# aligokalppeker/hypelcnn

Hardware: AMD Instinct MI355X
Metric: HSI+LiDAR patches/sec fwd+bwd (GRSS2013 7×7×145) at 1/2/4/8 GPU (higher is better)
Workload: dtype f32 (3 x bf16 split operands, 6 partial products, fp32 accumulate); 1 GPU; BASELINE.json configs[1]: GRSS2013 HYPELCNNModel, batch 1024 per GPU, fp32 HIP kernels; train step (fwd+bwd+TF1-Adam), 7x7 patch, 144 HSI + 1 LiDAR bands, 15 classes, alg_param_hypelcnn.json, random-init weights; batch_per_gpu=1024, global_batch=1024, parallelism=single, hip_graph=True

## Files before the change

### hypelcnn_amd/csrc/elementwise.hip

```cpp
#include <stdlib.h>

#include "common.h"


namespace {

constexpr int STAT_TX = 64;

struct EwShape {
    int tx_log2;
    int grid;
};
static inline EwShape ew_shape(int64_t rows, int cvec) {
    int l = 0;
    while ((1 << l) < cvec && l < 8) ++l;
    const int ty = 256 >> l;
    int64_t g = (rows + ty - 1) / ty;
    if (g < 1) g = 1;
    constexpr int cap = 8192;
    if (g > cap) g = cap;
    return EwShape{l, (int)g};
}
static inline bool aligned16(const void* p) { return p == nullptr || (((uintptr_t)p) & 15) == 0; }
static inline bool rows_v4(const void* p, int64_t ld) { return p == nullptr || (aligned16(p) && ld % 4 == 0); }
// ... 351 lines not shown
        const double unbiased = n_total > 1.0 ? m2 / (n_total - 1.0) : var;
        moving_mean[col] = (float)((double)moving_mean[col] * decay + mean_a * (1.0 - (double)decay));
        moving_var[col] = (float)((double)moving_var[col] * decay + unbiased * (1.0 - (double)decay));
    }
}

template <int VEC>
__global__ __launch_bounds__(256) void col_stats_partial_kernel(const float* __restrict__ x, int64_t ld, int64_t rows,
                                                                 int c, int chunk_rows, float* __restrict__ partial) {
    constexpr int TX = STAT_TX / VEC, TY = 256 / TX;
    __shared__ float sh[2][TY][STAT_TX];
    const int tx = threadIdx.x & (TX - 1), ty = threadIdx.x / TX;
    const int col = blockIdx.y * STAT_TX + tx * VEC;
    const int64_t r0 = (int64_t)blockIdx.x * chunk_rows;
    const int64_t r1 = min(rows, r0 + (int64_t)chunk_rows);
    Vec<VEC> s = {}, ss = {}, shift = {};
    if (col < c) {
        shift.load(x + r0 * ld + col);
#pragma unroll 4
        for (int64_t r = r0 + ty; r < r1; r += TY) {
            Vec<VEC> v;
            v.load(x + r * ld + col);
            vec_each<VEC>([&](int k) {
                const float d = v.v[k] - shift.v[k];
                s.v[k] += d;
                ss.v[k] += d * d;
            });
        }
    }
    s.store(&sh[0][ty][tx * VEC]);
    ss.store(&sh[1][ty][tx * VEC]);
    __syncthreads();
    const int cc = blockIdx.y * STAT_TX + threadIdx.x;
    if (threadIdx.x < STAT_TX && cc < c) {
        float ts = 0.0f, tss = 0.0f;
#pragma unroll
        for (int k = 0; k < TY; ++k) {
            ts += sh[0][k][threadIdx.x];
            tss += sh[1][k][threadIdx.x];
        }
        const float cnt = (float)(r1 - r0);
        const float mean_d = ts / cnt;
        float m2 = tss - ts * mean_d;
        if (m2 < 0.0f) m2 = 0.0f;
        float shift_cc;
        if constexpr (VEC == 1) shift_cc = shift.v[0];
        else shift_cc = x[r0 * ld + cc];
        float* po = partial + (int64_t)blockIdx.x * 2 * c;
        po[cc] = shift_cc + mean_d;
        po[c + cc] = m2;
    }
}

__global__ void rstd_from_var_kernel(const float* __restrict__ var, int c, float eps, float* __restrict__ rstd) {
    const int i = blockIdx.x * blockDim.x + threadIdx.x;
    if (i < c) rstd[i] = (float)(1.0 / sqrt((double)var[i] + (double)eps));
}

template <int VEC>
__global__ __launch_bounds__(256) void bn_act_fwd_kernel(
    const float* __restrict__ y, int64_t ldy, int64_t rows, int c, const float* __restrict__ mean,
    const float* __restrict__ rstd, const float* __restrict__ beta, int act, float alpha,
    const float* __restrict__ mask, int64_t ldm, const float* __restrict__ res1, int64_t ld1,
    const int32_t* __restrict__ idx1, const float* __restrict__ res2, int64_t ld2, const int32_t* __restrict__ idx2,
    float* __restrict__ z, int64_t ldz, int tx_log2) {
    ew_loop<VEC>(rows, c, tx_log2, [&](int64_t row, int col) {
        Vec<VEC> v;
        v.load(y + row * ldy + col);
        if (mean) {
            Vec<VEC> m, r, b;
            m.load_param(mean + col); r.load_param(rstd + col); b.load_param(beta + col);
#pragma unroll
            for (int k = 0; k < VEC; ++k) v.v[k] = hypel_bn_pre(hypel_bn_xhat(v.v[k], m.v[k], r.v[k]), b.v[k]);
        }
#pragma unroll
        for (int k = 0; k < VEC; ++k) v.v[k] = hypel_act(v.v[k], act, alpha);
        if (mask) {
            Vec<VEC> mk;
            mk.load(mask + row * ldm + col);
#pragma unroll
            for (int k = 0; k < VEC; ++k) v.v[k] *= mk.v[k];
        }
        if (res1) {
            if (idx1) {
#pragma unroll
                for (int k = 0; k < VEC; ++k) v.v[k] += res1[row * ld1 + idx1[col + k]];
            } else {
                Vec<VEC> t;
                t.load(res1 + row * ld1 + col);
#pragma unroll
                for (int k = 0; k < VEC; ++k) v.v[k] += t.v[k];
            }
        }
        if (res2) {
            if (idx2) {
#pragma unroll
                for (int k = 0; k < VEC; ++k) v.v[k] += res2[row * ld2 + idx2[col + k]];
            } else {
                Vec<VEC> t;
                t.load(res2 + row * ld2 + col);
#pragma unroll
                for (int k = 0; k < VEC; ++k) v.v[k] += t.v[k];
            }
        }
        v.store(z + row * ldz + col);
    });
// ... 727 lines not shown
                                            int32_t n_splits, int32_t accumulate, hypel_stream_t stream) {
    HYPEL_REQUIRE(partial0 && out0 && partial1 && out1 && n_splits >= 1 && count0 > 0 && count1 > 0,
                  "hypel_reduce_splits_pair_f32");
    if (n_splits >= 32 && count0 <= 65536 && count1 <= 65536) {
        hipLaunchKernelGGL(reduce_splits_wave_pair_kernel, dim3(hypel_grid_1d((count0 + count1) * 64, 256)), dim3(256), 0, ST,
                           partial0, stride0, count0, out0, partial1, stride1, count1, out1, n_splits, accumulate);
        HYPEL_CHECK_LAUNCH("hypel_reduce_splits_pair_f32");
        return 0;
    }
    int rc = hypel_reduce_splits_f32(partial0, stride0, n_splits, out0, count0, accumulate, nullptr, 0, 0, stream);
    if (rc == 0) rc = hypel_reduce_splits_f32(partial1, stride1, n_splits, out1, count1, accumulate, nullptr, 0, 0, stream);
    return rc;
}

extern "C" int hypel_reduce_splits_multi_f32(const float* base, const hypel_reduce_entry_t* entries, int32_t n_entries,
                                             hypel_stream_t stream) {
    HYPEL_REQUIRE(base && entries && n_entries >= 0, "hypel_reduce_splits_multi_f32");
    if (n_entries == 0) return 0;
    constexpr int gx = 768;
    hipLaunchKernelGGL(reduce_splits_multi_kernel, dim3(gx, n_entries), dim3(256), 0, ST, base, entries);
    HYPEL_CHECK_LAUNCH("hypel_reduce_splits_multi_f32");
    return 0;
}

extern "C" int hypel_reduce_splits_multi_sized_f32(const float* base, const hypel_reduce_entry_t* entries, int32_t n_entries,
                                                   int64_t max_count, hypel_stream_t stream) {
    HYPEL_REQUIRE(base && entries && n_entries >= 0 && max_count >= 0, "hypel_reduce_splits_multi_sized_f32");
    if (n_entries == 0 || max_count == 0) return 0;
    const int64_t want = (max_count + 4 * 256 - 1) / (4 * 256);
    const int gx = (int)(want < 1 ? 1 : (want > 768 ? 768 : want));
    hipLaunchKernelGGL(reduce_splits_multi_kernel, dim3(gx, n_entries), dim3(256), 0, ST, base, entries);
    HYPEL_CHECK_LAUNCH("hypel_reduce_splits_multi_sized_f32");
    return 0;
}

static int launch_col_stats(const float* x, int64_t ld, int64_t rows, int32_t c, int32_t chunk_rows, float* partial,
                            hypel_stream_t stream) {
    const int n_chunks = (int)((rows + chunk_rows - 1) / chunk_rows);
    const bool v4 = c % 4 == 0 && rows_v4(x, ld);
    hipLaunchKernelGGL(HYPEL_VEC_KERNEL(v4, col_stats_partial_kernel), dim3(n_chunks, (c + STAT_TX - 1) / STAT_TX), dim3(256),
                       0, ST, x, ld, rows, c, chunk_rows, partial);
    return 0;
}

extern "C" int hypel_col_stats_partial(const float* x, int64_t ld, int64_t rows, int32_t c, int32_t chunk_rows,
                                       float* partial, hypel_stream_t stream) {
    HYPEL_REQUIRE(x && partial && rows > 0 && c > 0 && chunk_rows > 0, "hypel_col_stats_partial");
    launch_col_stats(x, ld, rows, c, chunk_rows, partial,
                     stream);
    HYPEL_CHECK_LAUNCH("hypel_col_stats_partial");
    return 0;
}

extern "C" int hypel_bn_finalize(const float* partial, int32_t n_chunks, int32_t chunk_rows, int64_t rows, int32_t c,
                                 float eps, float* mean, float* rstd, float* moving_mean, float* moving_var,
                                 float decay, hypel_stream_t stream) {
    HYPEL_REQUIRE(partial && mean && rstd && n_chunks > 0 && c > 0, "hypel_bn_finalize");
    HYPEL_REQUIRE((moving_mean == nullptr) == (moving_var == nullptr), "hypel_bn_finalize");
    hipLaunchKernelGGL(bn_finalize_kernel, dim3((c + 15) / 16), dim3(256), 0, ST, partial, n_chunks, chunk_rows, rows,
                       c, eps, mean, rstd, moving_mean, moving_var, decay);
    HYPEL_CHECK_LAUNCH("hypel_bn_finalize");
    return 0;
}

extern "C" int hypel_bn_merge_partials(const float* partial, int32_t n_chunks, int32_t chunk_rows, int64_t rows,
                                       int32_t c, float* out, hypel_stream_t stream) {
    HYPEL_REQUIRE(partial && out && n_chunks > 0 && c > 0 && rows > 0, "hypel_bn_merge_partials");
    hipLaunchKernelGGL(bn_merge_partials_kernel, dim3((c + 15) / 16), dim3(256), 0, ST, partial, n_chunks, chunk_rows,
                       rows, c, out);
    HYPEL_CHECK_LAUNCH("hypel_bn_merge_partials");
    return 0;
}

extern "C" int hypel_bn_finalize_ranks(const float* gathered, int32_t world, int32_t c, float eps, float* mean,
                                       float* rstd, float* moving_mean, float* moving_var, float decay,
                                       hypel_stream_t stream) {
    HYPEL_REQUIRE(gathered && mean && rstd && world > 0 && c > 0, "hypel_bn_finalize_ranks");
    HYPEL_REQUIRE((moving_mean == nullptr) == (moving_var == nullptr), "hypel_bn_finalize_ranks");
    hipLaunchKernelGGL(bn_finalize_ranks_kernel, dim3((c + 63) / 64), dim3(64), 0, ST, gathered, world, c, eps, mean,
                       rstd, moving_mean, moving_var, decay);
    HYPEL_CHECK_LAUNCH("hypel_bn_finalize_ranks");
    return 0;
}

extern "C" int hypel_rstd_from_var(const float* var, int32_t c, float eps, float* rstd, hypel_stream_t stream) {
    HYPEL_REQUIRE(var && rstd && c > 0, "hypel_rstd_from_var");
    hipLaunchKernelGGL(rstd_from_var_kernel, dim3((c + 63) / 64), dim3(64), 0, ST, var, c, eps, rstd);
    HYPEL_CHECK_LAUNCH("hypel_rstd_from_var");
    return 0;
}

extern "C" int hypel_bn_act_fwd(const float* y, int64_t ldy, int64_t rows, int32_t c, const float* mean,
                                const float* rstd, const float* beta, int32_t act, float alpha, const float* mask,
                                int64_t ldm, const float* res1, int64_t ld1, const int32_t* idx1, const float* res2,
                                int64_t ld2, const int32_t* idx2, float* z, int64_t ldz, hypel_stream_t stream) {
    HYPEL_REQUIRE(y && z && rows > 0 && c > 0, "hypel_bn_act_fwd");
    HYPEL_REQUIRE((mean == nullptr) == (rstd == nullptr) && (mean == nullptr) == (beta == nullptr), "hypel_bn_act_fwd");
    const bool v4 = c % 4 == 0 && rows_v4(y, ldy) && rows_v4(z, ldz) && rows_v4(mask, ldm) &&
                    (idx1 || rows_v4(res1, ld1)) && (idx2 || rows_v4(res2, ld2));
    const EwShape sh = ew_shape(rows, v4 ? c / 4 : c);
    hipLaunchKernelGGL(HYPEL_VEC_KERNEL(v4, bn_act_fwd_kernel), dim3(sh.grid), dim3(256), 0, ST, y, ldy, rows, c, mean,
                       rstd, beta, act, alpha, mask, ldm, res1, ld1, idx1, res2, ld2, idx2, z, ldz, sh.tx_log2);
    HYPEL_CHECK_LAUNCH("hypel_bn_act_fwd");
    return 0;
}

// ... 273 lines not shown
```

### hypelcnn_amd/plan.py

```python
import os

import numpy as np

from . import abi, graph as G
from .backend import COPY_BLOCK_DTYPE, GEMM_BM, MTILE_DTYPE, REDUCE_ENTRY_DTYPE, SEG_DTYPE, Ref
from .gemm_tables import SEG_PAIR_FLAG, GemmTables, Launch

STAT_CHUNK_ROWS = 256
STAT_BLOCKS = 256


def stat_chunk_rows(rows):
    c = (rows + STAT_BLOCKS - 1) // STAT_BLOCKS
    c = max(16, min(STAT_CHUNK_ROWS, c))
    return (c + 3) // 4 * 4
WGRAD_ROW_CHUNK = 512
TARGET_BLOCKS = 1536
WGRAD_MAX_SPLITS = 64
WGRAD_MIN_SPLITS = 0
DGRAD_MAX_SEGS = 18
MAX_TAPS_PER_TILE = 9
L2_CHUNK_BYTES = int(3.5 * (1 << 20))
SPLITK_BELOW = 400
SPLITK_TARGET = 768
TAP_SPLIT_MIN_BATCH = 64


ACT_IN_GEMM = True
SMALL_BN_ROWS = 1024
MERGE_WGRAD = True


class Storage:

    def __init__(self, buf, nb, ld, pixmap, ch_off, c, npix):
        self.buf = buf
        self.nb = nb
        self.ld = ld
        self.pixmap = pixmap
        self.ch_off = ch_off
        self.c = c
        self.npix = npix

    def pix_off(self, p):
        q = p if self.pixmap is None else self.pixmap[p]
        return q * self.nb * self.ld + self.ch_off

    @property
    def contiguous(self):
        return self.pixmap is None

    @property
    def rows(self):
        return self.npix * self.nb


MSE_PARTIALS = abi.const("HYPEL_MSE_PARTIALS")
DP_SYNC_WORK = 0.5
DP_TWO_BUCKET_BYTES = int(float(os.environ.get("HYPEL_DP_TWO_BUCKET_MB", "1048576")) * (1 << 20))
DP_BUCKET_BYTES = int(float(os.environ.get("HYPEL_DP_BUCKET_MB", "256")) * (1 << 20))
DP_MAX_BUCKETS = 8
HINT_OVERRIDE = {k: int(v) for k, v in (kv.split("=") for kv in os.environ.get("HYPEL_HINT_OVERRIDE", "").split(",") if kv)}
RESIDENT_BLOCKS_64 = 6 * 256
GEMM_SINGLE_SEG = abi.const("HYPEL_GEMM_SINGLE_SEG")
GEMM_PAIRED_SEGS = abi.const("HYPEL_GEMM_PAIRED_SEGS")
GEMM_BK = 32
GEMM_SPLIT6 = abi.const("HYPEL_GEMM_SPLIT6")
GEMM_MULTI_SPLIT6 = abi.const("HYPEL_GEMM_MULTI_SPLIT6")
_gs = os.environ.get("HYPEL_GEMM_SPLIT", "6").split(":")
GEMM_SPLIT = int(_gs[0] or 0)
GEMM_SPLIT_WIDTH = int(_gs[1]) if len(_gs) > 1 else 0
GEMM_SPLIT_MIN_FLOPS = float(os.environ.get("HYPEL_GEMM_SPLIT_MIN_GFLOP", "2")) * 1e9
SPLIT_NOMINAL_BATCH = 1024
SPLIT_NOMINAL_BATCH_GAN = 4096
GEMM_SPLIT_MIN_N = 32
SPLIT_OVERRIDE = {k: int(v) for k, v in (kv.split("=") for kv in os.environ.get("HYPEL_SPLIT_OVERRIDE", "").split(",") if kv)}
KSLICE_MIN_GAIN = 0.10
KSLICE_OVERHEAD_K = 24
KSLICE_MIN_K = 48
KSLICE_MAX_SLICES = 16
KSLICE_FRAC_MIN = 0.7
KSLICE_REDUCE_COST_K = 55
KSLICE_SLOTS = {1: 768, 2: 512, 3: 512}
SPLIT6_BN = {1: 32, 2: 64, 3: 128}
GEMM_MFMA16X4 = abi.const("HYPEL_GEMM_MFMA16X4")
GEMM_VAR_N = abi.const("HYPEL_GEMM_VAR_N")
MERGE_LEVELS = set(x for x in os.environ.get("HYPEL_MERGE_LEVELS", "fwd,dgrad,wgrad").split(",") if x and x != "0")
MERGE_LEVELS_MAX_COUT = 64
MERGE_PASS_MAX_COUT = {"fwd": 16, "dgrad": 1 << 20, "wgrad": 1 << 20}
MERGE_WGRAD_MIN_COUT = 1
MERGE_WGRAD_MAX_COUT = 64
MERGE_FWD_MAX_COUT_SPLIT = 32
MERGE_MAX_TAPS = 0
MERGE_SPLIT_MAX_TAPS = 16
MERGE_SPLIT_KPARTS = False
MERGE_FWD_HINT = 2


for _kv in filter(None, os.environ.get("HYPEL_PLAN_SET", "").split(",")):
    _k, _, _v = _kv.partition("=")
    if not isinstance(globals().get(_k), (bool, int, float)) or _k.startswith("_"):
        raise ValueError(f"HYPEL_PLAN_SET: {_k!r} is not a numeric constant of hypelcnn_amd.plan")
    globals()[_k] = type(globals()[_k])(float(_v)) if not isinstance(globals()[_k], bool) else bool(int(_v))


class TowerPlan:

    _defer_bias_sums = False

    def __init__(self, tower, nb, session, loss=None, labels_c=None, external_masks=False, seed=1234, global_nb=None,
                 sync_bn=False):
        self.tower = tower
        self.nb = int(nb)
        self.global_nb = global_nb
        dist_ = getattr(session, "dist", None)
        self.sync_bn = bool(sync_bn) and dist_ is not None and tower.is_training
        self.world = dist_[0] if dist_ is not None else 1
        self.sess = session
        self.be = session.backend
        self.training = tower.is_training
        self.loss = loss
        self.external_masks = external_masks
        self.seed = seed
        self.buffers = {}
        self.tables = []
        self.storage = {}
        self.grad_written = {}
        self.fwd = []
        self.bwd = []
        self.node_aux = {}
        self.mask_bufs = {}
        self.scratch_sizes = {"scratch_partial": 1, "scratch_wgrad": 1, "sums": 2}
        self._pending_scratch = []
        self.param_written = set()
        self.sync_points = []
        self._level_layouts = {}
        self._pending_wgrads = []
        self._wgrad_flushes = 0
        self._kslice_bufs = 0
        self._build()

    def _trains(self, variables):
        return True

    def _needs_grad(self, t):
        return t.owner.needs_grad

    def _param_acc(self, var):
        acc = 1 if var.name in self.param_written else 0
# ... 561 lines not shown
        self.tables.append(t)
        self.fwd.insert(pos, Launch("copy_blocks_f32", (base, Ref(t), len(ents), max(e[2] * e[3] for e in ents)),
                                    nbytes=8 * sum(e[2] * e[3] for e in ents), tag="level-pack"))

    @staticmethod
    def _columns(node):
        cols, col = [], 0
        for b in node.branches:
            cols.append((b, col))
            col += b.cout
        return cols

    @staticmethod
    def _taps(branches, cin, lay=None):
        if lay is not None:
            C, col0 = lay["C"], lay["col0"]
            return [(dy, dx, d * cin * C + col0[r], col0[r], C - col0[r]) for d, (dy, dx, r) in enumerate(lay["offs"])]
        return [(i - (b.k - 1) // 2, j - (b.k - 1) // 2, b.w.offset + (i * b.k + j) * cin * b.cout, col, b.cout)
                for b, col in branches for i in range(b.k) for j in range(b.k)]

    @staticmethod
    def _fwd_segs(taps, s_st, h, w, p, wo=None, r=0):
        py, px = divmod(p, w if wo is None else wo)
        py, px = py + r, px + r
        return [(s_st.pix_off((py + dy) * w + px + dx), w_, s_st.c) for dy, dx, w_, _, _ in taps
                if 0 <= py + dy < h and 0 <= px + dx < w]

    @staticmethod
    def _valid_geometry(node):
        if not node.valid:
            return None, 0
        return node.out.hw[1], (node.branches[0].k - 1) // 2

    @staticmethod
    def _partial_copies(segs, S, kp_n=1, ldb=0):
        def cut(k, q):
            return k if q == kp_n else min(k, (k * q // kp_n + 15) // 16 * 16)

        for kp in range(kp_n):
            part = [(a + cut(k, kp), b + cut(k, kp) * ldb, cut(k, kp + 1) - cut(k, kp)) for a, b, k in segs]
            for si in range(S):
                yield kp, si, part[len(part) * si // S:len(part) * (si + 1) // S]

    @staticmethod
    def _channel_parts(cin, h, w):
        return max(1, min(4, -(-(h * w * GEMM_BM * cin * 4) // L2_CHUNK_BYTES), cin // 16))

    def _reduce_tap_copies(self, ybuf, rows, c, col, n, copies, bias=None):
        if copies > 1:
            self.fwd.append(Launch("reduce_splits_f32", (self._ref(ybuf, rows * c + col), rows * c, copies - 1,
                                                         self._ref(ybuf, col), rows * n, 1, bias, n, c),
                                   nbytes=4 * rows * n * (copies + 1), tag="tap-split-reduce"))

    def _fwd_level_merged(self, node, lay, s_st, ybuf, c, h, w):
        nb, C = self.nb, lay["C"]
        rows_all = node.out.npix * nb
        taps = self._taps(self._columns(node), lay["cin"], lay)
        rings = [[t for t, o in zip(taps, lay["offs"]) if o[2] == r] for r in range(lay["rmax"] + 1)]
        whole = GemmTables()
        for p in range(h * w):
            for ring in rings:
                whole.add_group(p * nb * c + ring[0][3], self._fwd_segs(ring, s_st, h, w, p), nb, n=ring[0][4])
        flags = GEMM_VAR_N | (GEMM_MFMA16X4 if lay["co"] <= 16 and C <= 64 else 0)
        tag = f"fwd:{node.branches[0].scope}/merged"
        sp6 = self._split6(tag, whole, C, 0, 0, flags, False)
        max_taps = MERGE_MAX_TAPS or (MERGE_SPLIT_MAX_TAPS if sp6 else MAX_TAPS_PER_TILE)
        S_r = [max(1, -(-len(ring) // max_taps)) for ring in rings]
        kp_n = self._channel_parts(lay["cin"], h, w) if not sp6 or MERGE_SPLIT_KPARTS else 1
        chunk0 = [sum(S_r[:r]) for r in range(len(rings) + 1)]
        if chunk0[-1] * kp_n > 1:
            self._alloc(ybuf, rows_all * c * chunk0[-1] * kp_n)
        tb = GemmTables()
        for gi, (c_off, segs, _) in enumerate(whole.groups):
            r = gi % len(rings)
            for kp, si, chunk in self._partial_copies(segs, S_r[r], kp_n, C):
                tb.add_group(((chunk0[r] + si) * kp_n + kp) * rows_all * c + c_off, chunk, nb, subkey=kp, n=whole.ns[gi])
        pos = len(self.fwd)
        self._emit_gemm(self.fwd, tb, C, self._ref(s_st.buf), s_st.ld, 0, self._ref(lay["buf"]), C, 0, self._ref(ybuf), c,
                        None, 0, tag, allow_split=False, hint=MERGE_FWD_HINT, flags=flags,
                        sp6=sp6)
        if len(self.fwd) > pos:
            self.fwd[pos].kparts = kp_n
        for b, col in self._columns(node):
            self._reduce_tap_copies(ybuf, rows_all, c, col, b.cout, chunk0[(b.k - 1) // 2 + 1] * kp_n)

    def _fwd_conv(self, node, aux, s_st, ybuf, c, h, w, bias_ref):
        nb, cin = self.nb, s_st.c
        rows_all = node.out.npix * nb
        splits = {}
        kparts = 1
        if nb >= TAP_SPLIT_MIN_BATCH:
            for b in node.branches:
                taps = min(b.k, h) * min(b.k, w)
                if taps > MAX_TAPS_PER_TILE:
                    splits[id(b)] = (taps + MAX_TAPS_PER_TILE - 1) // MAX_TAPS_PER_TILE
            if splits:
                kparts = self._channel_parts(cin, h, w)
                if kparts > 1:
                    for b in node.branches:
                        if b.k > 1:
                            splits[id(b)] = splits.get(id(b), 1) * kparts
        s_max = max(splits.values()) if splits else 1
        if s_max > 1:
            self._alloc(ybuf, rows_all * c * s_max)
        by_cout = {}
        for b, col in self._columns(node):
            by_cout.setdefault((b.cout, bias_ref is not None and splits.get(id(b), 1) > 1), []).append((b, col))
        fuse_stats = (node.has_bn and node.training and len(node.branches) == 1
                      and node.branches[0].k == 1 and s_st.contiguous and s_max == 1 and c > 16
                      and not self._small_bn(node, rows_all))
        aux["stats_in_gemm"] = fuse_stats
        for (cout, split_launch), items in by_cout.items():
            tb = GemmTables()
            kp_used = 1
            for b, col in items:
                if b.k == 1 and s_st.contiguous:
                    tb.add_group(col, [(s_st.pix_off(0), b.w.offset, cin)], rows_all)
                    continue
                S = splits.get(id(b), 1)
                kp_n = kparts if S >= kparts and S % kparts == 0 and kparts > 1 else 1
                kp_used = max(kp_used, kp_n)
                S_tap = S // kp_n
                taps = self._taps([(b, col)], cin)
                wo, vr = self._valid_geometry(node)
                for p in range(node.out.npix):
                    for kp, si, chunk in self._partial_copies(self._fwd_segs(taps, s_st, h, w, p, wo, vr), S_tap, kp_n,
                                                              cout):
                        tb.add_group((kp * S_tap + si) * rows_all * c + p * nb * c + col, chunk, nb, subkey=kp)
            pos = len(self.fwd)
            self._emit_gemm(self.fwd, tb, cout, self._ref(s_st.buf), s_st.ld, 0, Ref(self.sess.params), cout, 0,
                            self._ref(ybuf), c, None if split_launch else bias_ref, 0,
                            f"fwd:{items[0][0].scope}" + ("/split" if split_launch else ""), allow_split=False,
                            stats=((rows_all + GEMM_BM - 1) // GEMM_BM) * 2 * c if fuse_stats else None)
            if len(self.fwd) > pos:
                self.fwd[pos].kparts = kp_used
            for b, col in items:
                self._reduce_tap_copies(ybuf, rows_all, c, col, cout, splits.get(id(b), 1),
                                        None if bias_ref is None else bias_ref + col)

    def _fwd_linear(self, idx, node):
        nb = self.nb
        out = node.out
        c = node.cout
        aux = self._vec_params(node)
        self.node_aux[idx] = aux
        ybuf = f"y:{idx}"
        self._alloc(ybuf, out.npix * nb * c)
        y_st = Storage(ybuf, nb, c, None, 0, c, out.npix)
        aux["y"] = y_st
        bias_ref = self._p(aux["bias"]) if node.has_bias else None

        if node.kind == "conv":
            s_st = self.storage_of(node.sources[0])
            h, w = node.sources[0].hw
            lay = self._level_pass(idx, node, "fwd")
            if lay is not None:
                aux["stats_in_gemm"] = False
                self._fwd_level_merged(node, lay, s_st, ybuf, c, h, w)
            else:
                self._fwd_conv(node, aux, s_st, ybuf, c, h, w, bias_ref)
        elif node.kind == "blockdense":
            src = node.sources[0]
            s_st = self.storage_of(src)
            cout = node.branches[0].cout
            tb = GemmTables()
            for pi, (off, width) in enumerate(node.in_slices):
                tb.add_group(pi * cout, [(s_st.pix_off(0) + off, node.branches[pi].w.offset, width)], nb)
            act_flag = self._act_in_gemm(node, cout)
            aux["act_in_gemm"] = bool(act_flag)
            self._emit_gemm(self.fwd, tb, cout, self._ref(s_st.buf), s_st.ld, 0, Ref(self.sess.params), cout, 0,
                            self._ref(ybuf), c, bias_ref, 0, f"fwd:{node.branches[0].scope}+{len(node.branches) - 1}",
                            allow_split=False, flags=act_flag)
        else:
            b = node.branches[0]
            rowbase = 0
            for si, src in enumerate(node.sources):
                s_st = self.storage_of(src)
                tb = GemmTables()
                segs = [(s_st.pix_off(p), b.w.offset + (rowbase + p * src.c) * c, src.c) for p in range(src.npix)]
                tb.add_group(0, segs, nb)
                act_flag = 0
                if len(node.sources) == 1 and self._split_k(tb, c, s_st.ld, 0, c, 0, c) is None:
                    act_flag = self._act_in_gemm(node, c)
                aux["act_in_gemm"] = bool(act_flag)
                self._emit_gemm(self.fwd, tb, c, self._ref(s_st.buf), s_st.ld, 0, Ref(self.sess.params), c, 0,
                                self._ref(ybuf), c, bias_ref if si == 0 else None, 1 if si > 0 else 0,
                                f"fwd:{b.scope}",
                                flags=act_flag)
                rowbase += src.npix * src.c

        rows = out.npix * nb
        if node.has_bn:
            self._alloc(f"mean:{idx}", c)
            self._alloc(f"rstd:{idx}", c)
            if node.training and self._small_bn(node, rows):
                aux["small_bn"] = True
                aux["mean"] = self._ref(f"mean:{idx}")
            elif node.training and aux.get("stats_in_gemm"):
                n_chunks = (rows + GEMM_BM - 1) // GEMM_BM
                self._emit_bn_finalize(idx, node, aux, n_chunks, GEMM_BM, rows, c)
                aux["mean"] = self._ref(f"mean:{idx}")
            elif node.training:
                chunk = stat_chunk_rows(rows)
                n_chunks = (rows + chunk - 1) // chunk
                l1 = Launch("col_stats_partial", (self._ref(ybuf), c, rows, c, chunk, None),
                            nbytes=4 * rows * c, tag="bn-stats")
                self._scratch(l1, "partial", "scratch_partial", n_chunks * 2 * c)
                self.fwd.append(l1)
                self._emit_bn_finalize(idx, node, aux, n_chunks, chunk, rows, c)
                aux["mean"] = self._ref(f"mean:{idx}")
            else:
                self.fwd.append(Launch("rstd_from_var", (self._s(aux["mv"]), c, float(node.bn_eps),
                                                         self._ref(f"rstd:{idx}")), tag="bn-infer"))
                aux["mean"] = self._s(aux["mm"])
            aux["rstd"] = self._ref(f"rstd:{idx}")
            aux["beta_ref"] = self._p(aux["beta"])
        if node.has_post and aux.get("act_in_gemm"):
            self.storage[id(out)] = y_st
        elif node.has_post:
            zbuf = f"z:{idx}"
            self._alloc(zbuf, rows * c)
            self.storage[id(out)] = Storage(zbuf, nb, c, None, 0, c, out.npix)
            self._emit_post_fwd(idx, node, self._ref(ybuf), c, rows, c, aux, self._ref(zbuf))
        else:
            self.storage[id(out)] = y_st

    def _act_in_gemm(self, node, n):
        act = node.act
        if not (ACT_IN_GEMM and node.has_post and not node.has_bn and not node.residuals and node.dropout_keep is None
                and act is not None and act.code == 1 and n > 16 and not self.sync_bn):
            return 0
        for code, slope in ((1, 0.1), (2, 0.18), (3, 0.2), (4, 0.01)):
            if np.float32(act.alpha) == np.float32(slope):
                return code << 16
        return 0

    def _emit_bn_finalize(self, idx, node, aux, n_chunks, chunk, rows, c):
        mean_ref, rstd_ref = self._ref(f"mean:{idx}"), self._ref(f"rstd:{idx}")
        tail = (float(node.bn_eps), mean_ref, rstd_ref, self._s(aux["mm"]), self._s(aux["mv"]), self._bn_decay(node))
        if not self.sync_bn:
            l2 = Launch("bn_finalize", (None, n_chunks, chunk, rows, c) + tail, tag="bn-finalize")
            self._scratch(l2, "partial", "scratch_partial", n_chunks * 2 * c)
            self.fwd.append(l2)
            return
        rec = 2 * c + 1
        l2 = Launch("bn_merge_partials", (None, n_chunks, chunk, rows, c, None), tag="bn-sync-merge")
        self._scratch(l2, "partial", "scratch_partial", n_chunks * 2 * c)
        self._scratch(l2, "out", "sbn_local", rec)
        l3 = Launch("_allgather", (None, rec, None), tag="bn-sync-gather")
        self._scratch(l3, "src", "sbn_local", rec)
        self._scratch(l3, "dst", "sbn_all", self.world * rec)
        l4 = Launch("bn_finalize_ranks", (None, self.world, c) + tail, tag="bn-finalize")
        self._scratch(l4, "gathered", "sbn_all", self.world * rec)
        self.fwd += [l2, l3, l4]

    @staticmethod
    def _bn_decay(node):
        return float(node.bn_decay) if node.bn_update else 1.0

    def _mask_ref(self, idx, node, rows, c):
        if node.dropout_keep is None:
# ... 732 lines not shown
```

### include/hypel.h

```cpp
#ifndef HYPEL_H
#define HYPEL_H
#include <stdint.h>

#ifdef __cplusplus
extern "C" {
#endif

typedef void* hypel_stream_t;

#define HYPEL_ABI_VERSION 8

enum { HYPEL_ACT_NONE = 0, HYPEL_ACT_LRELU = 1, HYPEL_ACT_RELU = 2, HYPEL_ACT_SIGMOID = 3, HYPEL_ACT_TANH = 4 };

int hypel_version(void);
const char* hypel_last_error(void);
int hypel_device_info(int32_t* n_cu, int32_t* n_xcd);

uint32_t hypel_crc32c(uint32_t crc, const void* data, uint64_t n);

int hypel_nhwc_to_pnc(const float* x, float* out, int64_t n, int32_t p, int32_t c, int64_t ld,
                      hypel_stream_t stream);
int hypel_pnc_to_nhwc(const float* in, int64_t ld, float* x, int64_t n, int32_t p, int32_t c,
                      hypel_stream_t stream);
int hypel_fill_f32(float* dst, int64_t count, float value, hypel_stream_t stream);
// ... 25 lines not shown
                       float* c, int64_t ldc, int32_t n, const hypel_group_t* groups, const hypel_seg_t* segs,
                       const hypel_tile_t* tiles, int32_t n_tiles, const float* bias, int32_t accumulate,
                       hypel_stream_t stream);

int hypel_seg_gemm_stats_f32(const float* a, int64_t lda, int32_t trans_a, const float* b, int64_t ldb,
                             int32_t trans_b, float* c, int64_t ldc, int32_t n, const hypel_group_t* groups,
                             const hypel_seg_t* segs, const hypel_tile_t* tiles, int32_t n_tiles, const float* bias,
                             int32_t accumulate, float* stats_partial, hypel_stream_t stream);

int hypel_seg_gemm_res_f32(const float* a, int64_t lda, int32_t trans_a, const float* b, int64_t ldb, int32_t trans_b,
                           float* c, int64_t ldc, int32_t n, const hypel_group_t* groups, const hypel_seg_t* segs,
                           const hypel_tile_t* tiles, int32_t n_tiles, const float* bias, int32_t accumulate,
                           const float* res, int64_t ldr, const int32_t* res_start, hypel_stream_t stream);

typedef struct {
    int64_t c_off; int64_t a_off0; int64_t b_off0;
    int32_t m0; int32_t rows; int32_t n0; int32_t n;
    int32_t seg_begin; int32_t seg_count; int32_t k0; int32_t flags;
    int32_t lda; int32_t ldb; int32_t ldc; int32_t reserved;
} hypel_mtile_t;
int hypel_seg_gemm_multi_f32(const float* base, int32_t trans_a, int32_t trans_b, int32_t tile_width,
                             const hypel_seg_t* segs, const hypel_mtile_t* blocks, int32_t n_blocks,
                             hypel_stream_t stream);

typedef struct {
    int64_t partial_off; int64_t out_off; int64_t stride; int64_t count; int32_t n_splits; int32_t flags;
} hypel_reduce_entry_t;
int hypel_reduce_splits_multi_f32(const float* base, const hypel_reduce_entry_t* entries, int32_t n_entries,
                                  hypel_stream_t stream);
int hypel_reduce_splits_multi_sized_f32(const float* base, const hypel_reduce_entry_t* entries, int32_t n_entries,
                                        int64_t max_count, hypel_stream_t stream);

int hypel_reduce_splits_wave_multi_f32(const float* base, const hypel_reduce_entry_t* entries, int32_t n_entries,
                                       int64_t total_count, hypel_stream_t stream);

int hypel_reduce_splits_f32(const float* partial, int64_t stride, int32_t n_splits, float* out, int64_t count,
                            int32_t accumulate, const float* bias, int32_t n, int64_t ldc, hypel_stream_t stream);

int hypel_reduce_splits_pair_f32(const float* partial0, int64_t stride0, int64_t count0, float* out0,
                                 const float* partial1, int64_t stride1, int64_t count1, float* out1, int32_t n_splits,
                                 int32_t accumulate, hypel_stream_t stream);

typedef struct {
    int64_t src_off; int64_t dst_off; int32_t rows; int32_t cols; int32_t src_ld; int32_t dst_ld; int32_t flags;
    int32_t reserved;
} hypel_copy_block_t;
int hypel_copy_blocks_f32(const float* base, const hypel_copy_block_t* entries, int32_t n_entries,
                          int64_t max_block_elems, hypel_stream_t stream);
int hypel_copy_pair_f32(float* dst0, const float* src0, int64_t n0, float* dst1, const float* src1, int64_t n1,
                        hypel_stream_t stream);

int hypel_col_stats_partial(const float* x, int64_t ld, int64_t rows, int32_t c, int32_t chunk_rows, float* partial,
                            hypel_stream_t stream);
int hypel_bn_finalize(const float* partial, int32_t n_chunks, int32_t chunk_rows, int64_t rows, int32_t c, float eps,
                      float* mean, float* rstd, float* moving_mean, float* moving_var, float decay,
                      hypel_stream_t stream);
int hypel_bn_merge_partials(const float* partial, int32_t n_chunks, int32_t chunk_rows, int64_t rows, int32_t c,
                            float* out, hypel_stream_t stream);
int hypel_bn_finalize_ranks(const float* gathered, int32_t world, int32_t c, float eps, float* mean, float* rstd,
                            float* moving_mean, float* moving_var, float decay, hypel_stream_t stream);
int hypel_bn_act_small_fwd(const float* y, int64_t ldy, int64_t rows, int32_t c, float eps, const float* beta,
                           int32_t act, float alpha, const float* mask, int64_t ldm, float* mean, float* rstd,
                           float* moving_mean, float* moving_var, float decay, float* z, int64_t ldz,
                           hypel_stream_t stream);
int hypel_bn_act_small_bwd(const float* dz, int64_t lddz, const float* y, int64_t ldy, int64_t rows, int32_t c,
                           const float* mean, const float* rstd, const float* beta, int32_t act, float alpha,
                           const float* mask, int64_t ldm, float* dy, int64_t lddy, float* dparam,
                           int32_t accumulate, hypel_stream_t stream);
int hypel_rstd_from_var(const float* var, int32_t c, float eps, float* rstd, hypel_stream_t stream);

int hypel_bn_act_fwd(const float* y, int64_t ldy, int64_t rows, int32_t c, const float* mean, const float* rstd,
                     const float* beta, int32_t act, float alpha, const float* mask, int64_t ldm, const float* res1,
                     int64_t ld1, const int32_t* idx1, const float* res2, int64_t ld2, const int32_t* idx2, float* z,
                     int64_t ldz, hypel_stream_t stream);
int hypel_bn_act_bwd_reduce(const float* dz, int64_t lddz, const float* y, int64_t ldy, int64_t rows, int32_t c,
                            const float* mean, const float* rstd, const float* beta, int32_t act, float alpha,
                            const float* mask, int64_t ldm, int32_t chunk_rows, float* partial, hypel_stream_t stream);
int hypel_bwd_reduce_finalize(const float* partial, int32_t n_chunks, int32_t c, float* sums, float* dparam,
                              int32_t accumulate, hypel_stream_t stream);
int hypel_act_bias_bwd_reduce(const float* dz, int64_t lddz, const float* y, int64_t ldy, int64_t rows, int32_t c,
                              int32_t act, float alpha, const float* mask, int64_t ldm, int32_t chunk_rows, float* partial,
                              float* dy, int64_t lddy, hypel_stream_t stream);
int hypel_bn_act_bwd_apply(const float* dz, int64_t lddz, const float* y, int64_t ldy, int64_t rows, int32_t c,
                           const float* mean, const float* rstd, const float* beta, int32_t act, float alpha,
                           const float* mask, int64_t ldm, const float* sums, float* dy, int64_t lddy,
                           hypel_stream_t stream);
int hypel_bn_act_bwd_apply_global(const float* dz, int64_t lddz, const float* y, int64_t ldy, int64_t rows, int32_t c,
                                  const float* mean, const float* rstd, const float* beta, int32_t act, float alpha,
                                  const float* mask, int64_t ldm, const float* sums, int64_t stat_rows, float* dy,
                                  int64_t lddy, hypel_stream_t stream);
int hypel_chanmap_bwd(const float* dz, int64_t lddz, int64_t rows, int32_t c, float* dr, int64_t lddr, int32_t cin,
                      const int32_t* start, int32_t accumulate, hypel_stream_t stream);

int hypel_softmax_xent(const float* logits, int64_t ld, int64_t n, int32_t c, const float* labels, int64_t ldl,
                       float* loss, float* dlogits, int64_t lddl, float gscale, hypel_stream_t stream);
int hypel_mse(const float* a, int64_t lda, const float* b, int64_t ldb, int64_t rows, int32_t c, float* out, float* da,
              int64_t ldda, float gscale, float* ws, hypel_stream_t stream);
#define HYPEL_MSE_PARTIALS 1024
int hypel_mse_partial_f32(const float* a, int64_t lda, const float* b, int64_t ldb, int64_t rows, int32_t c, float* da,
                          int64_t ldda, float gscale, float* ws, hypel_stream_t stream);
int hypel_loss_finalize_f32(const float* loss_rows, int32_t n_rows, const float* mse_ws, double mse_scale, float* out_ce,
                            float* out_mse, float* flag, uint64_t* step, hypel_stream_t stream);

int hypel_sum_f32(const float* x, int64_t count, float scale, float* out, float* ws, hypel_stream_t stream);

int hypel_adam_tf1(float* p, const float* g, float* m, float* v, int64_t count, float lr_t, float beta1, float beta2,
// ... 278 lines not shown
```

### profiles/analyze_trace.py

```python
import csv, json, sys, os
sys.path.insert(0, os.path.dirname(os.path.dirname(os.path.abspath(__file__))))
import numpy as np
workload = "hypelcnn"
if "--workload" in sys.argv:
    i = sys.argv.index("--workload")
    workload = sys.argv[i + 1]
    del sys.argv[i:i + 2]
trace = sys.argv[1]
rows = list(csv.DictReader(open(trace)))
rows.sort(key=lambda r: int(r['Start_Timestamp']))
from tests.emu_backend import EmuBackend
import bench
nb = bench.CLASSIFIER_WORKLOADS[workload][5]
ctx, train_step, lr, alg = bench.build_model(nb, EmuBackend(), workload)
ctx.capture_graphs = False
ct = train_step.compiled(nb)
plan = ct.plan
launches = [l for l in plan.fwd + plan.bwd if l.name not in ('_fork','_join')]
names = []
for l in launches:
    names.append(l.name)
    if l.name in ("mse", "sum_f32"): names.append(l.name + "_fin")
kn = [r['Kernel_Name'] for r in rows]
starts = [i for i, k in enumerate(kn) if 'nhwc_to_pnc' in k]
i0 = starts[-1]
seq = rows[i0:]
def is_h(k): return 'anonymous namespace' in k
seq = [r for r in seq if is_h(r['Kernel_Name'])]
out = []
j = 0
for l in launches:
    n_k = 2 if l.name in ("mse", "sum_f32") else 1
    dur = 0
    for _ in range(n_k):
        r = seq[j]; j += 1
        dur += int(r['End_Timestamp']) - int(r['Start_Timestamp'])
    out.append((l.name, l.tag, l.flops, dur, r['Grid_Size_X'] if 'Grid_Size_X' in r else r.get('Grid_Size')))
tot = sum(o[3] for o in out)
print("total kernel ns per step", tot, " gemm ns", sum(o[3] for o in out if o[0].startswith('seg_gemm')))
print(f"{'name':18s} {'tag':34s} {'GFLOP':>8s} {'us':>8s} {'TF/s':>7s} grid")
for o in out:
    if o[3] > 20000 or (len(sys.argv) > 2 and sys.argv[2] == 'all'):
        tf = o[2]/o[3]/1e3 if o[2] else 0
        print(f"{o[0]:18s} {o[1]:34s} {o[2]/1e9:8.2f} {o[3]/1e3:8.1f} {tf:7.1f} {o[4]}")
bytag = {}
for o in out:
    key = o[0] if not o[0].startswith('seg_gemm') else 'gemm:' + o[1].split(':')[0]
    bytag.setdefault(key, [0, 0, 0]); bytag[key][0] += o[3]; bytag[key][1] += o[2]; bytag[key][2] += 1
for k, v in sorted(bytag.items(), key=lambda t: -t[1][0]):
    print(f"{k:28s} {v[0]/1e3:9.1f} us  n={v[2]:3d}  {v[1]/max(v[0],1)/1e3:6.1f} TF/s")
```

Measured before the change: 181,800 patches/s.

## Fuse tap-split partial reduction with BN column statistics in one kernel

Adds a level_reduce_stats kernel that sums the per-pixel split-K and tap-split partial copies, adds any deferred bias, writes the result back, and accumulates BN column sum and sum-of-squares partials in the same pass. The plan now emits this kernel in place of the separate reduce_splits launches plus col_stats_partial, and tracks a per-pixel copy count so pixels with fewer taps read fewer copies. The goal is to cut launches and avoid re-reading the conv output for statistics. The cost is a more complex kernel with per-pixel branching and count-table loads, which may diverge across lanes.

Measured after the change: 181,900 patches/s (median of 4 runs). Within noise of the previous version (+0.1%).

```diff
diff --git a/hypelcnn_amd/csrc/elementwise.hip b/hypelcnn_amd/csrc/elementwise.hip
--- a/hypelcnn_amd/csrc/elementwise.hip
+++ b/hypelcnn_amd/csrc/elementwise.hip
@@ -427,6 +427,146 @@
     }
 }
 
+constexpr int LEVEL_BURST = 8;
+template <int VEC>
+__global__ __launch_bounds__(256) void level_reduce_stats_kernel(float* y, int64_t ld, int64_t rows, int c,
+                                                                  int64_t copy_stride, int nb,
+                                                                  const int32_t* __restrict__ counts,
+                                                                  const float* __restrict__ bias,
+                                                                  const int32_t* __restrict__ bias_cols, int chunk_rows,
+                                                                  float* __restrict__ partial) {
+#pragma clang fp contract(off)
+    constexpr int TX = STAT_TX / VEC, TY = 256 / TX;
+    __shared__ float sh[2][TY][STAT_TX];
+    __shared__ float sh_shift[STAT_TX];
+    const int tx = threadIdx.x & (TX - 1), ty = threadIdx.x / TX;
+    const int col = blockIdx.y * STAT_TX + tx * VEC;
+    const int64_t r0 = (int64_t)blockIdx.x * chunk_rows;
+    const int64_t r1 = min(rows, r0 + (int64_t)chunk_rows);
+    const bool live = col < c;
+    Vec<VEC> b = {};
+    bool owed[VEC] = {};
+    if (live && bias)
+        vec_each<VEC>([&](int k) {
+            owed[k] = !bias_cols || bias_cols[col + k] != 0;
+            b.v[k] = owed[k] ? bias[col + k] : 0.0f;
+        });
+    struct Row {
+        Vec<VEC> p[LEVEL_BURST];
+        int cnt[VEC], smax;
+        float* yr;
+    };
+    int cnt[VEC], cnt_pix = -1, smax = 1;
+    auto request = [&](int64_t r, int pix, Row& w) {
+        if (pix != cnt_pix) {
+            cnt_pix = pix;
+            smax = 1;
+            vec_each<VEC>([&](int k) {
+                cnt[k] = counts[(int64_t)pix * c + col + k];
+                smax = max(smax, cnt[k]);
+            });
+        }
+        vec_each<VEC>([&](int k) { w.cnt[k] = cnt[k]; });
+        w.smax = smax;
+        w.yr = y + r * ld + col;
+#pragma unroll
+        for (int j = 0; j < LEVEL_BURST; ++j)
+            if (j < w.smax) w.p[j].load(w.yr + (int64_t)j * copy_stride);
+    };
+    auto finish = [&](Row& w, Vec<VEC>& v) {
+        Vec<VEC> t = b;
+#pragma unroll
+        for (int j = 1; j < LEVEL_BURST; ++j)
+            vec_each<VEC>([&](int k) {
+                if (j < w.cnt[k]) t.v[k] += w.p[j].v[k];
+            });
+        for (int j = LEVEL_BURST; j < w.smax; ++j) {
+            Vec<VEC> q;
+            q.load(w.yr + (int64_t)j * copy_stride);
+            vec_each<VEC>([&](int k) {
+                if (j < w.cnt[k]) t.v[k] += q.v[k];
+            });
+        }
+        bool changed = false;
+        vec_each<VEC>([&](int k) {
+            const bool keep = w.cnt[k] <= 1 && !owed[k];
+            v.v[k] = keep ? w.p[0].v[k] : t.v[k] + w.p[0].v[k];
+            changed |= !keep;
+        });
+        if (changed) v.store(w.yr);
+    };
+    Vec<VEC> s = {}, ss = {}, shift = {}, v0 = {};
+    auto accumulate = [&](const Vec<VEC>& v) {
+        vec_each<VEC>([&](int k) {
+            const float d = v.v[k] - shift.v[k];
+            s.v[k] += d;
+            if constexpr (VEC == 4) ss.v[k] = __builtin_fmaf(d, d, ss.v[k]);
+            else ss.v[k] += d * d;
+        });
+    };
+    int pix = (int)((r0 + ty) / nb);
+    int rem = (int)((r0 + ty) - (int64_t)pix * nb);
+    int64_t r = r0 + ty;
+    if (partial) {
+        if (live && ty == 0) {
+            Row w = {};
+            request(r0, pix, w);
+            finish(w, v0);
+            v0.store(&sh_shift[tx * VEC]);
+        }
+        __syncthreads();
+        if (live) {
+            shift.load(&sh_shift[tx * VEC]);
+            if (ty == 0) {
+                accumulate(v0);
+                r += TY;
+                for (rem += TY; rem >= nb; rem -= nb) ++pix;
+            }
+        }
+    }
+    if (live) {
+        for (; r + TY < r1; r += 2 * TY) {
+            Row w0 = {}, w1 = {};
+            Vec<VEC> v;
+            request(r, pix, w0);
+            for (rem += TY; rem >= nb; rem -= nb) ++pix;
+            request(r + TY, pix, w1);
+            for (rem += TY; rem >= nb; rem -= nb) ++pix;
+            finish(w0, v);
+            if (partial) accumulate(v);
+            finish(w1, v);
+            if (partial) accumulate(v);
+        }
+        if (r < r1) {
+            Row w = {};
+            Vec<VEC> v;
+            request(r, pix, w);
+            finish(w, v);
+            if (partial) accumulate(v);
+        }
+    }
+    if (!partial) return;
+    s.store(&sh[0][ty][tx * VEC]);
+    ss.store(&sh[1][ty][tx * VEC]);
+    __syncthreads();
+    const int cc = blockIdx.y * STAT_TX + threadIdx.x;
+    if (threadIdx.x < STAT_TX && cc < c) {
+        float ts = 0.0f, tss = 0.0f;
+#pragma unroll
+        for (int k = 0; k < TY; ++k) {
+            ts += sh[0][k][threadIdx.x];
+            tss += sh[1][k][threadIdx.x];
+        }
+        const float n_rows = (float)(r1 - r0);
+        const float mean_d = ts / n_rows;
+        float m2 = __builtin_fmaf(-ts, mean_d, tss);
+        if (m2 < 0.0f) m2 = 0.0f;
+        float* po = partial + (int64_t)blockIdx.x * 2 * c;
+        po[cc] = sh_shift[threadIdx.x] + mean_d;
+        po[c + cc] = m2;
+    }
+}
+
 __global__ void rstd_from_var_kernel(const float* __restrict__ var, int c, float eps, float* __restrict__ rstd) {
     const int i = blockIdx.x * blockDim.x + threadIdx.x;
     if (i < c) rstd[i] = (float)(1.0 / sqrt((double)var[i] + (double)eps));
@@ -1260,6 +1400,23 @@
     return 0;
 }
 
+extern "C" int hypel_level_reduce_stats_f32(float* y, int64_t ld, int64_t rows, int32_t c, int64_t copy_stride,
+                                            int32_t nb, int32_t npix, const int32_t* counts, const float* bias,
+                                            const int32_t* bias_cols, int32_t chunk_rows, float* partial,
+                                            hypel_stream_t stream) {
+    HYPEL_REQUIRE(y && counts && rows > 0 && c > 0 && ld >= c && chunk_rows > 0, "hypel_level_reduce_stats_f32");
+    HYPEL_REQUIRE(nb > 0 && npix > 0 && (int64_t)npix * nb == rows && copy_stride >= (rows - 1) * ld + c,
+                  "hypel_level_reduce_stats_f32");
+    HYPEL_REQUIRE(bias || !bias_cols, "hypel_level_reduce_stats_f32");
+    const int64_t n_chunks = (rows + chunk_rows - 1) / chunk_rows;
+    HYPEL_REQUIRE(n_chunks <= 0x7fffffff && (c + STAT_TX - 1) / STAT_TX <= 65535, "hypel_level_reduce_stats_f32");
+    const bool v4 = c % 4 == 0 && rows_v4(y, ld) && copy_stride % 4 == 0;
+    hipLaunchKernelGGL(HYPEL_VEC_KERNEL(v4, level_reduce_stats_kernel), dim3((unsigned)n_chunks, (c + STAT_TX - 1) / STAT_TX),
+                       dim3(256), 0, ST, y, ld, rows, c, copy_stride, nb, counts, bias, bias_cols, chunk_rows, partial);
+    HYPEL_CHECK_LAUNCH("hypel_level_reduce_stats_f32");
+    return 0;
+}
+
 extern "C" int hypel_bn_finalize(const float* partial, int32_t n_chunks, int32_t chunk_rows, int64_t rows, int32_t c,
                                  float eps, float* mean, float* rstd, float* moving_mean, float* moving_var,
                                  float decay, hypel_stream_t stream) {
diff --git a/hypelcnn_amd/plan.py b/hypelcnn_amd/plan.py
--- a/hypelcnn_amd/plan.py
+++ b/hypelcnn_amd/plan.py
@@ -3,7 +3,7 @@
 import numpy as np
 
 from . import abi, graph as G
-from .backend import COPY_BLOCK_DTYPE, GEMM_BM, MTILE_DTYPE, REDUCE_ENTRY_DTYPE, SEG_DTYPE, Ref
+from .backend import COPY_BLOCK_DTYPE, GEMM_BM, MTILE_DTYPE, REDUCE_ENTRY_DTYPE, SEG_DTYPE, SIGNATURES, Ref
 from .gemm_tables import SEG_PAIR_FLAG, GemmTables, Launch
 
 STAT_CHUNK_ROWS = 256
@@ -95,6 +95,9 @@
 MERGE_SPLIT_MAX_TAPS = 16
 MERGE_SPLIT_KPARTS = False
 MERGE_FWD_HINT = 2
+LEVEL_REDUCE_FUSED = True
+LEVEL_EVEN_CHUNKS_MIN_COUT = 1
+LEVEL_EVEN_CHUNKS_MAX_COUT = 0
 
 
 for _kv in filter(None, os.environ.get("HYPEL_PLAN_SET", "").split(",")):
@@ -762,11 +765,38 @@
                                                          self._ref(ybuf, col), rows * n, 1, bias, n, c),
                                    nbytes=4 * rows * n * (copies + 1), tag="tap-split-reduce"))
 
-    def _fwd_level_merged(self, node, lay, s_st, ybuf, c, h, w):
+    def _level_reduce_fused(self):
+        name = "level_reduce_stats_f32"
+        if not LEVEL_REDUCE_FUSED:
+            return False
+        return name in SIGNATURES if hasattr(self.be, "lib") else hasattr(self.be, "k_" + name)
+
+    @staticmethod
+    def _even_chunks(cout):
+        return LEVEL_EVEN_CHUNKS_MIN_COUT <= cout <= LEVEL_EVEN_CHUNKS_MAX_COUT
+
+    def _emit_level_reduce(self, lr, ybuf, rows, c, npix, chunk, n_stat_floats):
+        counts, owed, bias_ref = lr
+        t = self.be.upload(counts)
+        self.tables.append(t)
+        bias = cols = None
+        if bias_ref is not None and owed.any():
+            o_t = self.be.upload(owed)
+            self.tables.append(o_t)
+            bias, cols = bias_ref, Ref(o_t)
+        moved = int(counts.sum()) + int(((counts > 1) | (owed[None, :] != 0)).sum())
+        l = Launch("level_reduce_stats_f32", (self._ref(ybuf), c, rows, c, rows * c, self.nb, npix, Ref(t), bias, cols,
+                                              chunk, None), nbytes=4 * self.nb * moved, tag="tap-split-reduce")
+        if n_stat_floats:
+            self._scratch(l, "partial", "scratch_partial", n_stat_floats)
+        self.fwd.append(l)
+
+    def _fwd_level_merged(self, node, lay, s_st, ybuf, c, h, w, aux):
         nb, C = self.nb, lay["C"]
         rows_all = node.out.npix * nb
         taps = self._taps(self._columns(node), lay["cin"], lay)
         rings = [[t for t, o in zip(taps, lay["offs"]) if o[2] == r] for r in range(lay["rmax"] + 1)]
+        ring_col0 = [ring[0][3] for ring in rings]
         whole = GemmTables()
         for p in range(h * w):
             for ring in rings:
@@ -780,17 +810,31 @@
         chunk0 = [sum(S_r[:r]) for r in range(len(rings) + 1)]
         if chunk0[-1] * kp_n > 1:
             self._alloc(ybuf, rows_all * c * chunk0[-1] * kp_n)
+        fused = self._level_reduce_fused()
+        even = fused and self._even_chunks(lay["co"])
+        counts = np.ones((node.out.npix, c), np.int32)
         tb = GemmTables()
+        first = 0
         for gi, (c_off, segs, _) in enumerate(whole.groups):
             r = gi % len(rings)
-            for kp, si, chunk in self._partial_copies(segs, S_r[r], kp_n, C):
-                tb.add_group(((chunk0[r] + si) * kp_n + kp) * rows_all * c + c_off, chunk, nb, subkey=kp, n=whole.ns[gi])
+            S, base = S_r[r], chunk0[r]
+            if fused:
+                first = 0 if r == 0 else first
+                S, base = (-(-len(segs) // max_taps) if even else (S if segs else 0)), first
+                first += S
+                counts[gi // len(rings), ring_col0[r]:] = first * kp_n
+            for kp, si, chunk in self._partial_copies(segs, S, kp_n, C):
+                tb.add_group(((base + si) * kp_n + kp) * rows_all * c + c_off, chunk, nb, subkey=kp, n=whole.ns[gi])
         pos = len(self.fwd)
         self._emit_gemm(self.fwd, tb, C, self._ref(s_st.buf), s_st.ld, 0, self._ref(lay["buf"]), C, 0, self._ref(ybuf), c,
                         None, 0, tag, allow_split=False, hint=MERGE_FWD_HINT, flags=flags,
                         sp6=sp6)
         if len(self.fwd) > pos:
             self.fwd[pos].kparts = kp_n
+        if fused:
+            if counts.max() > 1:
+                aux["level_reduce"] = (counts, np.zeros(c, np.int32), None)
+            return
         for b, col in self._columns(node):
             self._reduce_tap_copies(ybuf, rows_all, c, col, b.cout, chunk0[(b.k - 1) // 2 + 1] * kp_n)
 
@@ -820,6 +864,8 @@
                       and node.branches[0].k == 1 and s_st.contiguous and s_max == 1 and c > 16
                       and not self._small_bn(node, rows_all))
         aux["stats_in_gemm"] = fuse_stats
+        fused = s_max > 1 and self._level_reduce_fused()
+        counts, owed = np.ones((node.out.npix, c), np.int32), np.zeros(c, np.int32)
         for (cout, split_launch), items in by_cout.items():
             tb = GemmTables()
             kp_used = 1
@@ -833,10 +879,13 @@
                 S_tap = S // kp_n
                 taps = self._taps([(b, col)], cin)
                 wo, vr = self._valid_geometry(node)
+                even = fused and id(b) in splits and self._even_chunks(cout)
                 for p in range(node.out.npix):
-                    for kp, si, chunk in self._partial_copies(self._fwd_segs(taps, s_st, h, w, p, wo, vr), S_tap, kp_n,
-                                                              cout):
-                        tb.add_group((kp * S_tap + si) * rows_all * c + p * nb * c + col, chunk, nb, subkey=kp)
+                    segs = self._fwd_segs(taps, s_st, h, w, p, wo, vr)
+                    S_p = max(1, -(-len(segs) // MAX_TAPS_PER_TILE)) if even else S_tap
+                    counts[p, col:col + cout] = kp_n * S_p
+                    for kp, si, chunk in self._partial_copies(segs, S_p, kp_n, cout):
+                        tb.add_group((kp * S_p + si) * rows_all * c + p * nb * c + col, chunk, nb, subkey=kp)
             pos = len(self.fwd)
             self._emit_gemm(self.fwd, tb, cout, self._ref(s_st.buf), s_st.ld, 0, Ref(self.sess.params), cout, 0,
                             self._ref(ybuf), c, None if split_launch else bias_ref, 0,
@@ -845,8 +894,13 @@
             if len(self.fwd) > pos:
                 self.fwd[pos].kparts = kp_used
             for b, col in items:
+                if fused:
+                    owed[col:col + cout] = int(split_launch)
+                    continue
                 self._reduce_tap_copies(ybuf, rows_all, c, col, cout, splits.get(id(b), 1),
                                         None if bias_ref is None else bias_ref + col)
+        if fused and (counts.max() > 1 or owed.any()):
+            aux["level_reduce"] = (counts, owed, bias_ref)
 
     def _fwd_linear(self, idx, node):
         nb = self.nb
@@ -866,7 +920,7 @@
             lay = self._level_pass(idx, node, "fwd")
             if lay is not None:
                 aux["stats_in_gemm"] = False
-                self._fwd_level_merged(node, lay, s_st, ybuf, c, h, w)
+                self._fwd_level_merged(node, lay, s_st, ybuf, c, h, w, aux)
             else:
                 self._fwd_conv(node, aux, s_st, ybuf, c, h, w, bias_ref)
         elif node.kind == "blockdense":
@@ -900,6 +954,11 @@
                 rowbase += src.npix * src.c
 
         rows = out.npix * nb
+        lr = aux.pop("level_reduce", None)
+        lr_stats = (lr is not None and node.has_bn and node.training and not self._small_bn(node, rows)
+                    and not aux.get("stats_in_gemm"))
+        if lr is not None and not lr_stats:
+            self._emit_level_reduce(lr, ybuf, rows, c, out.npix, stat_chunk_rows(rows), 0)
         if node.has_bn:
             self._alloc(f"mean:{idx}", c)
             self._alloc(f"rstd:{idx}", c)
@@ -913,10 +972,13 @@
             elif node.training:
                 chunk = stat_chunk_rows(rows)
                 n_chunks = (rows + chunk - 1) // chunk
-                l1 = Launch("col_stats_partial", (self._ref(ybuf), c, rows, c, chunk, None),
-                            nbytes=4 * rows * c, tag="bn-stats")
-                self._scratch(l1, "partial", "scratch_partial", n_chunks * 2 * c)
-                self.fwd.append(l1)
+                if lr_stats:
+                    self._emit_level_reduce(lr, ybuf, rows, c, out.npix, chunk, n_chunks * 2 * c)
+                else:
+                    l1 = Launch("col_stats_partial", (self._ref(ybuf), c, rows, c, chunk, None),
+                                nbytes=4 * rows * c, tag="bn-stats")
+                    self._scratch(l1, "partial", "scratch_partial", n_chunks * 2 * c)
+                    self.fwd.append(l1)
                 self._emit_bn_finalize(idx, node, aux, n_chunks, chunk, rows, c)
                 aux["mean"] = self._ref(f"mean:{idx}")
             else:
diff --git a/include/hypel.h b/include/hypel.h
--- a/include/hypel.h
+++ b/include/hypel.h
@@ -101,6 +101,9 @@
 
 int hypel_col_stats_partial(const float* x, int64_t ld, int64_t rows, int32_t c, int32_t chunk_rows, float* partial,
                             hypel_stream_t stream);
+int hypel_level_reduce_stats_f32(float* y, int64_t ld, int64_t rows, int32_t c, int64_t copy_stride, int32_t nb,
+                                 int32_t npix, const int32_t* counts, const float* bias, const int32_t* bias_cols,
+                                 int32_t chunk_rows, float* partial, hypel_stream_t stream);
 int hypel_bn_finalize(const float* partial, int32_t n_chunks, int32_t chunk_rows, int64_t rows, int32_t c, float eps,
                       float* mean, float* rstd, float* moving_mean, float* moving_var, float decay,
                       hypel_stream_t stream);
diff --git a/profiles/analyze_trace.py b/profiles/analyze_trace.py
--- a/profiles/analyze_trace.py
+++ b/profiles/analyze_trace.py
@@ -10,7 +10,9 @@
 rows = list(csv.DictReader(open(trace)))
 rows.sort(key=lambda r: int(r['Start_Timestamp']))
 from tests.emu_backend import EmuBackend
+from tests import emu_level_reduce
 import bench
+setattr(EmuBackend, emu_level_reduce.NAME, emu_level_reduce.k_level_reduce_stats_f32)
 nb = bench.CLASSIFIER_WORKLOADS[workload][5]
 ctx, train_step, lr, alg = bench.build_model(nb, EmuBackend(), workload)
 ctx.capture_graphs = False
```
